# simensov/ml4ca

Hardware: AMD Instinct MI355X
Metric: env-steps/sec at 65536 parallel envs (higher is better)
Workload: dtype f32

## Files before the change

ml4ca_amd/csrc/dpenv_env_dev.h:

```cpp
#ifndef DPENV_ENV_DEV_H
#define DPENV_ENV_DEV_H
#include <hip/hip_runtime.h>
#include <hip/hip_bf16.h>
#include <stdint.h>

#include "dpenv_dev.h"

namespace dpenv {

constexpr float kPi = 3.14159265358979323846f;

__device__ __forceinline__ void philox4x32_10(uint32_t c0, uint32_t c1, uint32_t c2, uint32_t c3, uint32_t k0,
                                              uint32_t k1, uint32_t out[4])
{
#pragma unroll
    for (int r = 0; r < 10; ++r) {
        const uint64_t p0 = (uint64_t)c0 * 0xD2511F53ull, p1 = (uint64_t)c2 * 0xCD9E8D57ull;
        const uint32_t hi0 = (uint32_t)(p0 >> 32), lo0 = (uint32_t)p0, hi1 = (uint32_t)(p1 >> 32), lo1 = (uint32_t)p1;
        const uint32_t n0 = hi1 ^ c1 ^ k0, n2 = hi0 ^ c3 ^ k1;
        c0 = n0; c1 = lo1; c2 = n2; c3 = lo0;
        k0 += 0x9E3779B9u; k1 += 0xBB67AE85u;
    }
    out[0] = c0; out[1] = c1; out[2] = c2; out[3] = c3;
}
// ... 533 lines not shown
        if (live) {
            if (a.obs_bf16) {
                uint16_t* p = (uint16_t*)dst;
#pragma unroll
                for (int k = 0; k < OD; ++k) p[(int64_t)k * n + i] = f2bf(o[k]);
            } else {
                float* p = (float*)dst;
#pragma unroll
                for (int k = 0; k < OD; ++k) p[(int64_t)k * n + i] = o[k];
            }
        }
        return;
    }
    lds_order<BLOCK>();
#pragma unroll
    for (int k = 0; k < OD; ++k) lds[tid * OD + k] = o[k];
    lds_order<BLOCK>();
    const int64_t base = (int64_t)blockIdx.x * (BLOCK * OD);
    const int64_t rem = (int64_t)n * OD - base;
    store_rows<OD, BLOCK>(dst, base, rem, a.obs_bf16, lds, tid);
}

struct Env {
    float N, E, psi, u, v, r;
    float refN, refE, refPsi;
    float pt[3];
    float ang[3];
    int steps;
    float sn, cs;
};

struct StepOut {
    float o[9];
    float reward;
    float parts[4];
    uint32_t d;
};

struct Wrench {
    float thr[3];
    float tx, ty, tn;
};

template <int MODE, bool DEFER_ANG = false>
__device__ __forceinline__ void env_decode_cmd(float ang[3], const float* act, float thr[3])
{
    thr[0] = clipf(act[0] * 100.0f, 100.0f);
    thr[1] = clipf(act[1] * 100.0f, 100.0f);
    thr[2] = clipf(act[2] * 100.0f, 100.0f);
    if (MODE == MODE_FULL) {
        ang[0] = clipf(act[3] * kPi, kPi); ang[1] = clipf(act[4] * kPi, kPi); ang[2] = clipf(act[5] * kPi, kPi);
    } else if (MODE == MODE_LIMITED) {
        ang[1] = clipf(act[3] * (kPi * 0.5f), kPi * 0.5f); ang[2] = clipf(act[4] * (kPi * 0.5f), kPi * 0.5f);
    } else if (MODE == MODE_FINAL_WRAP) {
        const float w3 = act[3] - 2.0f * floorf((act[3] + 1.0f) * 0.5f);
        const float w4 = act[4] - 2.0f * floorf((act[4] + 1.0f) * 0.5f);
        ang[1] = clipf(w3 * kPi, kPi); ang[2] = clipf(w4 * kPi, kPi);
    } else if (MODE == MODE_FINAL_CONT) {
        if (!DEFER_ANG) { ang[1] = clipf(atan2_lean(act[3], act[4]), kPi); ang[2] = clipf(atan2_lean(act[5], act[6]), kPi); }
    }
}

template <int MODE, bool DEFER_ANG = false>
__device__ __forceinline__ void env_decode(const Vessel& ve, float ang[3], const float* act, Wrench& w, const ThrustLoss* tl = nullptr)
{
    env_decode_cmd<MODE, DEFER_ANG>(ang, act, w.thr);
    if (MODE == MODE_FINAL_CONT) {
        float sc[4];
        const float np2 = fmaf(act[3], act[3], act[4] * act[4]), ns2 = fmaf(act[5], act[5], act[6] * act[6]);
        const float ip = __builtin_amdgcn_rsqf(np2), is = __builtin_amdgcn_rsqf(ns2);
        sc[0] = (np2 > 0.0f) ? act[3] * ip : 0.0f; sc[1] = (np2 > 0.0f) ? act[4] * ip : 1.0f;
        sc[2] = (ns2 > 0.0f) ? act[5] * is : 0.0f; sc[3] = (ns2 > 0.0f) ? act[6] * is : 1.0f;
        thrust_map(ve, w.thr, ang, w.tx, w.ty, w.tn, sc, tl);
    } else {
        thrust_map(ve, w.thr, ang, w.tx, w.ty, w.tn, nullptr, tl);
    }
}

__device__ __forceinline__ void env_plant(const StepArgs& a, const Vessel& ve, float tx, float ty, float tn, bool cur, float vcN,
                                          float vcE, float& N, float& E, float& psi, float& u, float& v, float& r, float sn, float cs)
{
    if (cur) {
        u -= fmaf(cs, vcN, sn * vcE);
        v -= fmaf(cs, vcE, -(sn * vcN));
    }
    const float h = a.h;
    const float hA = h * ve.inv11, h22 = h * ve.i22, h23 = h * ve.i23, h33 = h * ve.i33;
    const float yur = ve.Yur + ve.m11;
    const float nuv = ve.Nuv - ve.m11;
    const int nsub = a.hold_plant ? 0 : a.n_substeps;
    float aN = 0.0f, aE = 0.0f;
#pragma unroll 10
    for (int k = 0; k < nsub; ++k) {
        const float q = fmaf(ve.m22, v, ve.m23 * r);
        float fx = fmaf(-fmaf(ve.Xuu, fabsf(u), ve.Xu), u, tx);
        fx = fmaf(q, r, fx);
        float fy = fmaf(-fmaf(ve.Yvv, fabsf(v), ve.Yv), v, ty);
        fy = fmaf(-fmaf(yur, u, ve.Yr), r, fy);
        float fn = fmaf(-q, u, tn);
        fn = fmaf(-fmaf(nuv, u, ve.Nv), v, fn);
        fn = fmaf(-fmaf(ve.Nrr, fabsf(r), ve.Nr), r, fn);
        u = fmaf(hA, fx, u);
        v = fmaf(h22, fy, fmaf(h23, fn, v));
        r = fmaf(h23, fy, fmaf(h33, fn, r));
        aN = fmaf(-sn, v, fmaf(cs, u, aN));
        aE = fmaf(cs, v, fmaf(sn, u, aE));
        const float d = h * r;
        const float e = -0.5f * d;
        psi += d;
        const float c2 = fmaf(fmaf(e, cs, -sn), d, cs);
        const float s2n = fmaf(fmaf(e, sn, cs), d, sn);
        cs = c2; sn = s2n;
    }
    N = fmaf(h, aN, N);
    E = fmaf(h, aE, E);
    if (cur) {
        const float hn = h * (float)nsub;
        N = fmaf(hn, vcN, N);
        E = fmaf(hn, vcE, E);
    }
}

__device__ __forceinline__ void env_plant_finish(bool cur, float vcN, float vcE, float se, float ce, float& u, float& v)
{
    if (cur) {
        u += fmaf(ce, vcN, se * vcE);
        v += fmaf(ce, vcE, -(se * vcN));
    }
}

template <int MODE, bool EXT>
__device__ __forceinline__ void env_reward(const StepArgs& a, const float* o, const float thr[3], const float pt_old[3],
                                           const float ang_new[3], const float ang_prev[3], StepOut& out)
{
    float p_der = 0.0f;
    const float p_vel = -sqrt_hw(fmaf(o[3] * o[3], 0.5f, fmaf(o[4] * o[4], 0.5f, o[5] * o[5])));
    const float rr2 = fmaf(o[0], o[0], o[1] * o[1]);
    const float yaw = o[2] * (180.0f / kPi);
    const float multivar = 2.0f * __builtin_amdgcn_exp2f((-0.5f * 1.4426950408889634f) * fmaf(yaw * yaw, 1.0f / 25.0f, rr2));
    const float special = sqrt_hw(fmaf(yaw * 0.25f, yaw * 0.25f, rr2));
    const float p_pos = multivar + fmaxf(-1.0f, fmaf(-0.1f, special, 1.0f)) + 0.5f;
    const float p_thr = -(fabsf(thr[0]) * 0.20f + fabsf(thr[1]) * 0.30f + fabsf(thr[2]) * 0.30f) * 0.01f;
    if (EXT) {
        const float inv_dt = a.inv_dt;
        float pen = 0.0f;
#pragma unroll
        for (int k = 0; k < 3; ++k) pen -= fabsf((thr[k] - pt_old[k]) * inv_dt * 0.01f) * 0.05f;
        const float inv_bnd = (MODE == MODE_LIMITED) ? (2.0f / kPi) : (1.0f / kPi);
        const float angpen = -(fabsf((ang_new[1] - ang_prev[1]) * inv_dt * inv_bnd) * 0.01f +
                               fabsf((ang_new[2] - ang_prev[2]) * inv_dt * inv_bnd) * 0.01f);
        p_der = pen + fmaxf(-1.0f, angpen);
    }
    out.parts[0] = p_vel; out.parts[1] = p_pos; out.parts[2] = p_thr; out.parts[3] = p_der;
    out.reward = p_vel + p_pos + p_thr + p_der;
}

template <int MODE>
__device__ __forceinline__ void env_done(const StepArgs& a, Env& s, const float* act, const float* o, const float thr[3], bool has_ref,
                                         float nrN, float nrE, float nrP, StepOut& out)
{
    uint32_t d = 0;
    if (a.terminate) {
        float b[6];
        ss_bounds<MODE>(b);
        bool t = false;
#pragma unroll
        for (int k = 0; k < 6; ++k) t = t || (fabsf(o[k]) > b[k]);
        d = t ? DONE_TERMINAL : 0u;
    }
    {
        float chk = s.N + s.E + s.psi + s.u + s.v + s.r;
#pragma unroll
        for (int k = 0; k < ModeTraits<MODE>::A; ++k) chk += act[k];
        if (!(fabsf(chk) <= 3.0e38f)) d |= DONE_TERMINAL | DONE_FAULT;
    }
    if (has_ref) { s.refN = nrN; s.refE = nrE; s.refPsi = nrP; }
    s.steps += 1;
    if (a.max_ep_len > 0 && s.steps >= a.max_ep_len) d |= DONE_TIMELIMIT;
    s.pt[0] = thr[0]; s.pt[1] = thr[1]; s.pt[2] = thr[2];
    out.d = d;
}

struct StepRest {
    float thr[3], pt_old[3], ang_prev[3], ang_new[3];
};

template <int MODE, bool EXT, bool DEFER>
__device__ __forceinline__ void env_step_chain(const StepArgs& a, const Vessel& ve, Env& s, const float* act, bool has_ref,
                                               float nrN, float nrE, float nrP, bool cur, float vcN, float vcE, StepOut& out, StepRest& rest,
                                               int il = -1)
{
#pragma unroll
    for (int k = 0; k < 3; ++k) { rest.ang_prev[k] = s.ang[k]; rest.pt_old[k] = s.pt[k]; }
    Wrench w;
    if (il == IL_SHARED || (il >= 0 && thrust_loss_on(a))) {
        ThrustLoss tl;
        if (il == IL_SHARED) {
#pragma unroll
            for (int k = 0; k < 3; ++k) { tl.klf[k] = a.kl[k]; tl.klr[k] = a.kl[3 + k]; }
        } else {
            const float4 q0 = a.env_tab[(int64_t)ENV_GROUPS * a.env_stride + il], q1 = a.env_tab[(int64_t)(ENV_GROUPS + 1) * a.env_stride + il];
            tl.klf[0] = q0.x; tl.klf[1] = q0.y; tl.klf[2] = q0.z; tl.klr[0] = q0.w; tl.klr[1] = q1.x; tl.klr[2] = q1.y;
        }
        tl.u = s.u; tl.v = s.v; tl.r = s.r;
        if (cur) {
            tl.u -= fmaf(s.cs, vcN, s.sn * vcE);
            tl.v -= fmaf(s.cs, vcE, -(s.sn * vcN));
        }
        env_decode<MODE, DEFER>(ve, s.ang, act, w, &tl);
    } else {
        env_decode<MODE, DEFER>(ve, s.ang, act, w);
    }
#pragma unroll
    for (int k = 0; k < 3; ++k) { rest.thr[k] = w.thr[k]; rest.ang_new[k] = s.ang[k]; }
    float N = s.N, E = s.E, psi = s.psi, u = s.u, v = s.v, r = s.r;
    env_plant(a, ve, w.tx, w.ty, w.tn, cur, vcN, vcE, N, E, psi, u, v, r, s.sn, s.cs);
    const bool deg = (a.wrap_mode == WRAP_REFERENCE);
    float* o = out.o;
    bool same;
    float se, ce;
    {
        make_obs(N, E, psi, 0.0f, 0.0f, 0.0f, s.refN, s.refE, s.refPsi, rest.pt_old, deg, o, se, ce, same);
        if (!same) sincos_lean(psi, se, ce);
    }
    env_plant_finish(cur, vcN, vcE, se, ce, u, v);
    o[3] = u; o[4] = v; o[5] = r;
    s.N = N; s.E = E; s.psi = psi; s.u = u; s.v = v; s.r = r;
    s.sn = se; s.cs = ce;
    env_done<MODE>(a, s, act, o, rest.thr, has_ref, nrN, nrE, nrP, out);
}

template <int MODE, bool EXT, bool DEFER>
__device__ __forceinline__ void env_step_finish(const StepArgs& a, Env& s, const float* act, StepRest& rest, bool untouched, StepOut& out)
{
    if (DEFER && MODE == MODE_FINAL_CONT) {
        rest.ang_new[1] = clipf(atan2_lean(act[3], act[4]), kPi);
        rest.ang_new[2] = clipf(atan2_lean(act[5], act[6]), kPi);
        if (untouched) { s.ang[1] = rest.ang_new[1]; s.ang[2] = rest.ang_new[2]; }
    }
    env_reward<MODE, EXT>(a, out.o, rest.thr, rest.pt_old, rest.ang_new, rest.ang_prev, out);
}

template <int MODE, bool EXT>
__device__ __forceinline__ void env_step(const StepArgs& a, const Vessel& ve, Env& s, const float* act, bool has_ref,
                                         float nrN, float nrE, float nrP, bool cur, float vcN, float vcE, StepOut& out, int il = -1)
{
    StepRest rest;
    env_step_chain<MODE, EXT, false>(a, ve, s, act, has_ref, nrN, nrE, nrP, cur, vcN, vcE, out, rest, il);
    env_step_finish<MODE, EXT, false>(a, s, act, rest, true, out);
}

struct ResetDraw {
    float eta[3], nu[3], pt[3];
};

template <int MODE>
__device__ __forceinline__ void reset_draw(const StepArgs& a, int64_t gid, uint32_t episode, ResetDraw& d)
{
    sample_reset<MODE>(a, gid, episode, d.eta, d.nu);
    d.pt[0] = d.pt[1] = d.pt[2] = 0.0f;
    if (a.reset_acts) sample_reset_thrust(a, gid, episode, d.pt);
}

template <int MODE>
__device__ __forceinline__ void reset_apply(const StepArgs& a, Env& s, const ResetDraw& d, float o_new[9])
{
    s.N = d.eta[0]; s.E = d.eta[1]; s.psi = d.eta[2]; s.u = d.nu[0]; s.v = d.nu[1]; s.r = d.nu[2];
    s.pt[0] = d.pt[0]; s.pt[1] = d.pt[1]; s.pt[2] = d.pt[2];
    default_angles<MODE>(s.ang[0], s.ang[1], s.ang[2]);
    s.steps = 0;
    bool same;
    make_obs(s.N, s.E, s.psi, s.u, s.v, s.r, s.refN, s.refE, s.refPsi, s.pt, a.wrap_mode == WRAP_REFERENCE, o_new, s.sn, s.cs,
             same);
    if (!same) sincos_lean(s.psi, s.sn, s.cs);
}

template <int MODE>
__device__ __forceinline__ void env_auto_reset(const StepArgs& a, Env& s, int64_t gid, uint32_t episode, float o_new[9])
{
    ResetDraw d;
    reset_draw<MODE>(a, gid, episode, d);
    reset_apply<MODE>(a, s, d, o_new);
}

__device__ __forceinline__ void load_env(const float4* S0, const float4* S1, const float4* S2, const float4* RF, int il, Env& s)
{
    const float4 s0 = S0[il], s1 = S1[il], s2 = S2[il], rf = RF[il];
    s.N = s0.x; s.E = s0.y; s.psi = s0.z; s.u = s0.w; s.v = s1.x; s.r = s1.y;
    s.ang[0] = rf.w; s.ang[1] = s1.z; s.ang[2] = s1.w;
    s.pt[0] = s2.x; s.pt[1] = s2.y; s.pt[2] = s2.z; s.steps = __float_as_int(s2.w);
    s.refN = rf.x; s.refE = rf.y; s.refPsi = rf.z;
}

__device__ __forceinline__ void load_env(const StepArgs& a, int il, Env& s) { load_env(a.S0, a.S1, a.S2, a.RF, il, s); }

__device__ __forceinline__ void store_env(const StepArgs& a, int i, const Env& s, bool rf_dirty)
{
    a.S0[i] = make_float4(s.N, s.E, s.psi, s.u);
    a.S1[i] = make_float4(s.v, s.r, s.ang[1], s.ang[2]);
    a.S2[i] = make_float4(s.pt[0], s.pt[1], s.pt[2], __int_as_float(s.steps));
    if (rf_dirty) a.RF[i] = make_float4(s.refN, s.refE, s.refPsi, s.ang[0]);
}

}

#endif
```

ml4ca_amd/csrc/dpenv_kernels.hip:

```cpp
#include "dpenv_env_dev.h"

namespace dpenv {

#ifdef DPENV_STEP_TRACE
__device__ uint32_t* g_step_trace = nullptr;
constexpr int STEP_TRACE_RING = 8;
#endif

constexpr int RESETW_FIELDS = 18;
constexpr int RESETW_FIELDS_RND = 20;

template <int MODE>
__device__ __forceinline__ void reset_wave(const StepArgs& a, float* lds, int lane, int blk)
{
    const int n = a.n;
    const int i = blk * 64 + lane;
    const int il = i < n ? i : n - 1;
    const uint32_t ep = (uint32_t)a.episode[il];
    const float4 rf = a.RF[il];
    Env s;
    s.refN = rf.x; s.refE = rf.y; s.refPsi = rf.z;
    if (a.new_ref) { s.refN = a.new_ref[il]; s.refE = a.new_ref[(int64_t)n + il]; s.refPsi = a.new_ref[2 * (int64_t)n + il]; }
    ResetDraw d;
    reset_draw<MODE>(a, a.env_id_base + i, ep, d);
    float o[9];
    reset_apply<MODE>(a, s, d, o);
    lds[0 * 64 + lane] = s.N; lds[1 * 64 + lane] = s.E; lds[2 * 64 + lane] = s.psi;
#pragma unroll
    for (int k = 0; k < 9; ++k) lds[(3 + k) * 64 + lane] = o[k];
    lds[12 * 64 + lane] = s.pt[0]; lds[13 * 64 + lane] = s.pt[1]; lds[14 * 64 + lane] = s.pt[2];
    lds[15 * 64 + lane] = s.sn; lds[16 * 64 + lane] = s.cs;
    lds[17 * 64 + lane] = __uint_as_float(ep);
}

template <int MODE>
__device__ __forceinline__ void reset_from_lds(const float* lds, int lane, Env& s, float o_new[9])
{
    s.N = lds[0 * 64 + lane]; s.E = lds[1 * 64 + lane]; s.psi = lds[2 * 64 + lane];
#pragma unroll
    for (int k = 0; k < 9; ++k) o_new[k] = lds[(3 + k) * 64 + lane];
    s.u = o_new[3]; s.v = o_new[4]; s.r = o_new[5];
    s.pt[0] = lds[12 * 64 + lane]; s.pt[1] = lds[13 * 64 + lane]; s.pt[2] = lds[14 * 64 + lane];
    default_angles<MODE>(s.ang[0], s.ang[1], s.ang[2]);
    s.steps = 0;
    s.sn = lds[15 * 64 + lane]; s.cs = lds[16 * 64 + lane];
}

template <int MODE, bool EXT, int VES, bool RESETW = false>
__global__ __launch_bounds__(RESETW ? 2 * BLOCK : BLOCK) void step_kernel(const StepArgs a)
{
    const float4 *pS0 = a.S0, *pS1 = a.S1, *pS2 = a.S2, *pRF = a.RF;
    const float* paction = a.action;
    const int pn = a.n, playout = a.action_layout;
    constexpr int A = ModeTraits<MODE>::A;
    constexpr int OD = EXT ? 9 : 6;
    constexpr bool PER_CLASS = VES == VES_CLASS_LDS;
    constexpr bool RND = VES == VES_ENV_RND;
    constexpr bool ENV_VGPR = VES == VES_ENV_VGPR || RND;
    constexpr int IL = VES == VES_ARGS_LOSS ? IL_SHARED : IL_NONE;
    constexpr bool CURR = RND || VES == VES_ARGS_LOSS;
    static_assert(!RESETW || BLOCK == 64, "the reset wave pairs with ONE env wave");
    static_assert(VES != VES_ENV_LDS || BLOCK == 64, "the LDS-DMA image is [group][lane] of one wave");
    __shared__ float lds_io[BLOCK * 9];
    __shared__ float lds_cls[PER_CLASS ? VD_COUNT * MAX_CLASSES : 1];
    __shared__ float4 lds_pe[VES == VES_ENV_LDS ? ENV_GROUPS * 64 : 1];
    __shared__ float lds_rst[RESETW ? (CURR ? RESETW_FIELDS_RND : RESETW_FIELDS) * 64 : 1];
    __shared__ uint32_t lds_fin[RESETW ? 64 : 1];

    if (RESETW && threadIdx.x >= BLOCK) {
        const int lane = threadIdx.x - BLOCK;
        reset_wave<MODE>(a, lds_rst, lane, blockIdx.x);
        float4 hull[DRAW_GROUPS];
        const int i = blockIdx.x * 64 + lane;
        const bool rnd = RND && a.rand_tab != nullptr;
        if (rnd)
            draw_env_groups(hull_key(a), a.env_id_base + i, __float_as_uint(lds_rst[17 * 64 + lane]), [&](int g, const float4& q) { hull[g] = q; });
        if (CURR && a.cur_nom) {
            const float2 cd = current_draw(a, i, i < a.n ? i : a.n - 1, __float_as_uint(lds_rst[17 * 64 + lane]));
            lds_rst[18 * 64 + lane] = cd.x; lds_rst[19 * 64 + lane] = cd.y;
        }
        __syncthreads();
        if (rnd && lds_fin[lane] != 0u) {
#pragma unroll
            for (int g = 0; g < DRAW_GROUPS; ++g) store_draw_group(a.env_tab, a.env_stride, i, g, hull[g]);
        }
        return;
    }
    const int tid = threadIdx.x;
    const int i = blockIdx.x * BLOCK + tid;
    const int n = pn;
    const bool live = i < n;
    const int il = live ? i : n - 1;
#ifdef DPENV_STEP_TRACE
    const uint64_t trace_t0 = wall_clock64();
#endif

    float act[A];
    if (playout == LAYOUT_AOS) {
        const int64_t base = (int64_t)blockIdx.x * (BLOCK * A);
        load_rows<A, BLOCK>(paction + base, (int64_t)n * A - base, tid, act);
    } else {
#pragma unroll
        for (int k = 0; k < A; ++k) act[k] = paction[(int64_t)k * n + il];
    }
    Env s;
    load_env(pS0, pS1, pS2, pRF, il, s);
    float nrN = 0.0f, nrE = 0.0f, nrP = 0.0f;
    if (a.new_ref) { nrN = a.new_ref[il]; nrE = a.new_ref[(int64_t)n + il]; nrP = a.new_ref[2 * (int64_t)n + il]; }
    Current cur = {0.0f, 0.0f, 0.0f, 0.0f, 0u};
    float vc0 = 0.0f, beta0 = 0.0f;
    if (a.cur_vc) {
        cur.vc = a.cur_vc[il]; cur.beta = a.cur_beta[il];
        if (a.current_drift) { vc0 = a.cur_vc0[il]; beta0 = a.cur_beta0[il]; cur.ctr = a.drift_ctr[il]; }
    }
    int cls = 0;
    if (PER_CLASS) cls = a.class_id[il];
    Vessel ve_env;
    if (ENV_VGPR) ve_env = vessel_from_env(a.env_tab, a.env_stride, il);
    if (VES == VES_ENV_LDS) {
#pragma unroll
        for (int g = 0; g < ENV_GROUPS; ++g)
            __builtin_amdgcn_global_load_lds((const __attribute__((address_space(1))) void*)(a.env_tab + ((int64_t)g * a.env_stride + il)),
                                             (__attribute__((address_space(3))) void*)(lds_pe + g * 64), 16, 0, 0);
    }
    __builtin_amdgcn_sched_barrier(0);
    sincos_lean(s.psi, s.sn, s.cs);
    if (a.cur_vc) current_components(cur);
    if (PER_CLASS) {
        for (int k = tid; k < VD_COUNT * a.n_classes; k += BLOCK) {
            const int c = k / VD_COUNT, p = k - c * VD_COUNT;
            lds_cls[p * a.n_classes + c] = a.class_tab[k];
        }
    }
    if (playout == LAYOUT_AOS) {
#pragma unroll
        for (int j = 0; j < A; ++j) lds_io[j * BLOCK + tid] = act[j];
    }
    if (playout == LAYOUT_AOS || PER_CLASS) lds_order<BLOCK>();
    if (playout == LAYOUT_AOS) {
#pragma unroll
        for (int k = 0; k < A; ++k) act[k] = lds_io[tid * A + k];
    }
    if (VES == VES_ENV_LDS) {
        asm volatile("s_waitcnt vmcnt(0)" ::: "memory");
        __builtin_amdgcn_wave_barrier();
    }
    const Vessel ve = ENV_VGPR ? ve_env : VES == VES_ENV_LDS ? vessel_from_env_lds(lds_pe, tid)
                    : PER_CLASS ? vessel_from_lds(lds_cls, a.n_classes, cls) : vessel_from_args(a.v0);

    StepOut out;
    StepRest rest;
    env_step_chain<MODE, EXT, false>(a, ve, s, act, a.new_ref != nullptr, nrN, nrE, nrP, a.cur_vc != nullptr, cur.vcN, cur.vcE, out, rest, RND ? il : IL);
    bool rf_dirty = (a.new_ref != nullptr) || (MODE == MODE_FULL);
#ifdef DPENV_STEP_TRACE
    const bool early = false;
#else
    const bool early = !RESETW && !a.auto_reset;
#endif
    if (early) {
        if (live) {
            if (EXT && a.S3) a.S3[i] = make_float4(out.o[6], out.o[7], out.o[8], 0.0f);
            store_env(a, i, s, rf_dirty);
            a.done[i] = (uint8_t)out.d;
        }
        __builtin_amdgcn_sched_barrier(0);
        store_obs<OD>(a, a.obs, out.o, i, live, lds_io);
        __builtin_amdgcn_sched_barrier(0);
    }
    env_step_finish<MODE, EXT, false>(a, s, act, rest, true, out);
    if (a.current_drift) {
        current_drift_step(a, cur, vc0, beta0, a.env_id_base + i);
        if (live) { a.cur_vc[i] = cur.vc; a.cur_beta[i] = cur.beta; a.drift_ctr[i] = cur.ctr; }
    }
    if (early) {
        if (live) {
            a.rew[i] = out.reward;
            if (a.parts) {
                a.parts[i] = out.parts[0]; a.parts[(int64_t)n + i] = out.parts[1];
                a.parts[2 * (int64_t)n + i] = out.parts[2]; a.parts[3 * (int64_t)n + i] = out.parts[3];
            }
        }
        return;
    }

    float o_next[9];
#pragma unroll
    for (int k = 0; k < 9; ++k) o_next[k] = out.o[k];

    if (RESETW) {
        lds_fin[tid] = (a.auto_reset && out.d != 0u && live) ? 1u : 0u;
        __syncthreads();
    }
    if (a.auto_reset && out.d != 0u && live) {
        if (a.final_obs) {
            for (int k = 0; k < OD; ++k) {
                const int64_t idx = (a.obs_layout == LAYOUT_SOA) ? (int64_t)k * n + i : (int64_t)i * OD + k;
                if (a.obs_bf16) ((uint16_t*)a.final_obs)[idx] = f2bf(out.o[k]);
                else ((float*)a.final_obs)[idx] = out.o[k];
            }
        }
        const uint32_t ep = RESETW ? __float_as_uint(lds_rst[17 * 64 + tid]) : (uint32_t)a.episode[i];
        a.episode[i] = (int)(ep + 1u);
        if (RESETW) {
            reset_from_lds<MODE>(lds_rst, tid, s, o_next);
            if (CURR && a.cur_nom) {
                const float v = lds_rst[18 * 64 + tid], b = lds_rst[19 * 64 + tid];
                a.cur_vc[i] = v; a.cur_beta[i] = b; a.cur_vc0[i] = v; a.cur_beta0[i] = b;
            }
        } else {
            env_auto_reset<MODE>(a, s, a.env_id_base + i, ep, o_next);
            if (RND && a.rand_tab) redraw_vessel_table(a, i, ep);
            if (CURR && a.cur_nom) {
                const float2 cd = current_draw(a, i, i, ep);
                a.cur_vc[i] = cd.x; a.cur_beta[i] = cd.y; a.cur_vc0[i] = cd.x; a.cur_beta0[i] = cd.y;
            }
        }
        rf_dirty = true;
    }

    if (live) {
        if (EXT && a.S3) a.S3[i] = make_float4(o_next[6], o_next[7], o_next[8], 0.0f);
        store_env(a, i, s, rf_dirty);
        a.rew[i] = out.reward;
        a.done[i] = (uint8_t)out.d;
        if (a.parts) {
            a.parts[i] = out.parts[0]; a.parts[(int64_t)n + i] = out.parts[1];
            a.parts[2 * (int64_t)n + i] = out.parts[2]; a.parts[3 * (int64_t)n + i] = out.parts[3];
        }
    }
    __builtin_amdgcn_sched_barrier(0);
    store_obs<OD>(a, a.obs, o_next, i, live, lds_io);
#ifdef DPENV_STEP_TRACE
    if (tid == 0 && g_step_trace) {
        const uint64_t t1 = wall_clock64();
        const uint32_t slot = (uint32_t)(s.steps - 1) % STEP_TRACE_RING;
        uint32_t* rec = g_step_trace + ((size_t)slot * gridDim.x + blockIdx.x) * 4;
        rec[0] = __builtin_amdgcn_s_getreg((31 << 11) | 20);
        rec[1] = __builtin_amdgcn_s_getreg((31 << 11) | 4);
        rec[2] = (uint32_t)trace_t0;
        rec[3] = (uint32_t)t1;
    }
#endif
}

template <int MODE, bool EXT, int VES>
__global__ __launch_bounds__(RBLOCK) void rollout_kernel(const StepArgs a, const RolloutArgs ra)
{
    constexpr int A = ModeTraits<MODE>::A;
    constexpr int OD = EXT ? 9 : 6;
    constexpr bool PER_CLASS = VES == VES_CLASS_LDS, RND = VES == VES_ENV_RND, PER_ENV = VES == VES_ENV_VGPR || RND;
    constexpr int IL = VES == VES_ARGS_LOSS ? IL_SHARED : IL_NONE;
    constexpr bool CURR = RND || VES == VES_ARGS_LOSS;
    __shared__ float lds_act[RBLOCK * 7];
    __shared__ float lds_obs[RBLOCK * 9];
    __shared__ float lds_cls[PER_CLASS ? VD_COUNT * MAX_CLASSES : 1];

    const int tid = threadIdx.x;
    const int i = blockIdx.x * RBLOCK + tid;
    const int n = a.n;
    const bool live = i < n;
    const int il = live ? i : n - 1;

    Env s;
    load_env(a, il, s);
    sincos_lean(s.psi, s.sn, s.cs);
    Current cur = {0.0f, 0.0f, 0.0f, 0.0f, 0u};
    float vc0 = 0.0f, beta0 = 0.0f;
    if (a.cur_vc) {
        cur.vc = a.cur_vc[il]; cur.beta = a.cur_beta[il];
        if (a.current_drift) { vc0 = a.cur_vc0[il]; beta0 = a.cur_beta0[il]; cur.ctr = a.drift_ctr[il]; }
        current_components(cur);
    }
    int cls = 0;
    if (PER_CLASS) {
        cls = a.class_id[il];
        for (int k = tid; k < VD_COUNT * a.n_classes; k += RBLOCK) {
            const int c = k / VD_COUNT, p = k - c * VD_COUNT;
            lds_cls[p * a.n_classes + c] = a.class_tab[k];
        }
        lds_order<RBLOCK>();
    }
    Vessel ve = PER_ENV ? vessel_from_env(a.env_tab, a.env_stride, il)
                        : (PER_CLASS ? vessel_from_lds(lds_cls, a.n_classes, cls) : vessel_from_args(a.v0));
    if (!PER_CLASS && !PER_ENV) pin_vessel_in_vgprs(ve);
    uint32_t episode = a.auto_reset ? (uint32_t)a.episode[il] : 0u;
    bool ep_dirty = false, rf_dirty = (MODE == MODE_FULL);

    const int64_t step_stride_act = (int64_t)n * A;
    const int64_t step_stride_obs = (int64_t)n * OD;
    const int64_t blk_act = (int64_t)blockIdx.x * (RBLOCK * A);
    const int64_t blk_obs = (int64_t)blockIdx.x * (RBLOCK * OD);

    float pre[A];
    auto fetch = [&](int t) {
        const float* src = ra.actions + (int64_t)t * step_stride_act;
        if (a.action_layout == LAYOUT_AOS) {
            load_rows<A, RBLOCK>(src + blk_act, step_stride_act - blk_act, tid, pre);
        } else {
#pragma unroll
            for (int k = 0; k < A; ++k) pre[k] = src[(int64_t)k * n + il];
        }
    };
    fetch(0);
    int next_switch = 0;
    bool cur_dirty = false;
    float lag[3] = {0.0f, 0.0f, 0.0f};
    for (int t = 0; t < ra.T; ++t) {
        float act[A];
        if (a.action_layout == LAYOUT_AOS) {
            lds_order<RBLOCK>();
#pragma unroll
            for (int j = 0; j < A; ++j) lds_act[j * RBLOCK + tid] = pre[j];
            lds_order<RBLOCK>();
#pragma unroll
            for (int k = 0; k < A; ++k) act[k] = lds_act[tid * A + k];
        } else {
#pragma unroll
            for (int k = 0; k < A; ++k) act[k] = pre[k];
        }
        if (t + 1 < ra.T) fetch(t + 1);

        bool has_ref = false;
        float nrN = 0.0f, nrE = 0.0f, nrP = 0.0f;
        if (next_switch < ra.n_switch && ra.switch_step[next_switch] == t) {
            const float* rp = ra.refs + (int64_t)next_switch * 3 * n;
            nrN = rp[il]; nrE = rp[(int64_t)n + il]; nrP = rp[2 * (int64_t)n + il];
            has_ref = true; rf_dirty = true;
            ++next_switch;
        }
        StepOut out;
        env_step<MODE, EXT>(a, ve, s, act, has_ref, nrN, nrE, nrP, a.cur_vc != nullptr, cur.vcN, cur.vcE, out, RND ? il : IL);
        if (a.current_drift) current_drift_step(a, cur, vc0, beta0, a.env_id_base + i);
        float o_next[9];
#pragma unroll
        for (int k = 0; k < 9; ++k) o_next[k] = out.o[k];
        if (a.auto_reset && out.d != 0u && live) {
            env_auto_reset<MODE>(a, s, a.env_id_base + i, episode, o_next);
            if (RND && a.rand_tab) redraw_vessel(a, i, episode, ve);
            if (CURR && a.cur_nom) { current_redraw_inline(a, i, episode, cur, vc0, beta0); cur_dirty = true; }
            ++episode; ep_dirty = true; rf_dirty = true;
        }
        lag[0] = o_next[6]; lag[1] = o_next[7]; lag[2] = o_next[8];
        if (live) {
            (ra.rew + (int64_t)t * n)[(unsigned)i] = out.reward;
            (ra.done + (int64_t)t * n)[(unsigned)i] = (uint8_t)out.d;
        }
        if (a.obs_layout == LAYOUT_SOA) {
            if (live) {
#pragma unroll
                for (int k = 0; k < OD; ++k) {
                    const int64_t idx = (int64_t)t * step_stride_obs + (int64_t)k * n + i;
                    if (a.obs_bf16) ((uint16_t*)ra.obs)[idx] = f2bf(o_next[k]);
                    else ((float*)ra.obs)[idx] = o_next[k];
                }
            }
        } else {
            lds_order<RBLOCK>();
#pragma unroll
            for (int k = 0; k < OD; ++k) lds_obs[tid * OD + k] = o_next[k];
            lds_order<RBLOCK>();
            store_rows<OD, RBLOCK>(ra.obs, (int64_t)t * step_stride_obs + blk_obs, step_stride_obs - blk_obs, a.obs_bf16,
                                   lds_obs, tid);
        }
    }
    if (live) {
        store_env(a, i, s, rf_dirty);
        if (EXT) a.S3[i] = make_float4(lag[0], lag[1], lag[2], 0.0f);
        if (ep_dirty) a.episode[i] = (int)episode;
        if (a.current_drift) { a.cur_vc[i] = cur.vc; a.cur_beta[i] = cur.beta; a.drift_ctr[i] = cur.ctr; }
        if (CURR && cur_dirty) store_current(a, i, cur, vc0, beta0, true);
    }
// ... 307 lines not shown
        float o[9];
        float sr_, cr_;
        bool same_;
        make_obs(s0.x, s0.y, s0.z, s0.w, s1.x, s1.y, rf.x, rf.y, rf.z, pt, a.wrap_mode == WRAP_REFERENCE, o, sr_, cr_, same_);
        store_obs<OD>(a, a.obs, o, i, live, lds_io);
    }
}

__global__ __launch_bounds__(BLOCK) void get_state_kernel(const StepArgs a, float* st, int32_t* ctr)
{
    const int i = blockIdx.x * BLOCK + threadIdx.x;
    const int64_t n = a.n;
    if (i >= a.n) return;
    const float4 s0 = a.S0[i], s1 = a.S1[i], s2 = a.S2[i], rf = a.RF[i];
    if (st) {
        st[0 * n + i] = s0.x; st[1 * n + i] = s0.y; st[2 * n + i] = s0.z;
        st[3 * n + i] = s0.w; st[4 * n + i] = s1.x; st[5 * n + i] = s1.y;
        st[6 * n + i] = rf.x; st[7 * n + i] = rf.y; st[8 * n + i] = rf.z;
        st[9 * n + i] = s2.x; st[10 * n + i] = s2.y; st[11 * n + i] = s2.z;
        st[12 * n + i] = rf.w; st[13 * n + i] = s1.z; st[14 * n + i] = s1.w;
    }
    if (ctr) { ctr[i] = __float_as_int(s2.w); ctr[n + i] = a.episode[i]; }
}

__global__ __launch_bounds__(BLOCK) void set_state_kernel(const StepArgs a, const float* st, const int32_t* ctr)
{
    const int i = blockIdx.x * BLOCK + threadIdx.x;
    const int64_t n = a.n;
    if (i >= a.n) return;
    float4 s2 = a.S2[i];
    if (st) {
        a.S0[i] = make_float4(st[0 * n + i], st[1 * n + i], st[2 * n + i], st[3 * n + i]);
        a.S1[i] = make_float4(st[4 * n + i], st[5 * n + i], st[13 * n + i], st[14 * n + i]);
        a.RF[i] = make_float4(st[6 * n + i], st[7 * n + i], st[8 * n + i], st[12 * n + i]);
        s2.x = st[9 * n + i]; s2.y = st[10 * n + i]; s2.z = st[11 * n + i];
        a.S3[i] = make_float4(s2.x * 0.01f, s2.y * 0.01f, s2.z * 0.01f, 0.0f);
    }
    if (ctr) { s2.w = __int_as_float(ctr[i]); a.episode[i] = ctr[n + i]; }
    a.S2[i] = s2;
}

__global__ __launch_bounds__(BLOCK) void pack_env_vessels_kernel(const float* raw, int64_t p_stride, int64_t i_stride, float4* tab, uint32_t* loss_flag,
                                                                 int stride, int n)
{
    const int i = blockIdx.x * BLOCK + threadIdx.x;
    if (i >= n) return;
    float r[RAND_NPARAM], d[ENV_BLOCK_FLOATS];
#pragma unroll
    for (int p = 0; p < RAND_NPARAM; ++p) r[p] = raw[p * p_stride + i * i_stride];
    derive_env_block(r, d);
    store_env_block(tab, stride, i, d);
    const bool bad = !(d[0] == d[0]);
    const float nanv = __builtin_nanf("");
    tab[(int64_t)ENV_GROUPS * stride + i] = bad ? make_float4(nanv, nanv, nanv, nanv) : make_float4(r[26], r[27], r[28], r[29]);
    tab[(int64_t)(ENV_GROUPS + 1) * stride + i] = bad ? make_float4(nanv, nanv, 0.0f, 0.0f) : make_float4(r[30], r[31], 0.0f, 0.0f);
    bool any = false;
#pragma unroll
    for (int p = 26; p < RAND_NPARAM; ++p) any = any || (r[p] != 0.0f);
    if (loss_flag && __ballot(any) != 0ull && (threadIdx.x & 63) == __builtin_ctzll(__ballot(true))) atomicOr(loss_flag, 1u);
}

__global__ __launch_bounds__(BLOCK) void unpack_env_vessels_kernel(const float4* tab, int stride, float* out, int n)
{
    const int i = blockIdx.x * BLOCK + threadIdx.x;
    if (i >= n) return;
    float d[ENV_BLOCK_FLOATS];
#pragma unroll
    for (int g = 0; g < ENV_GROUPS; ++g) {
        const float4 q = tab[(int64_t)g * stride + i];
        d[4 * g] = q.x; d[4 * g + 1] = q.y; d[4 * g + 2] = q.z; d[4 * g + 3] = q.w;
    }
    float r[32];
    r[0] = d[VD_M11]; r[1] = d[VD_M22]; r[2] = d[VD_M23]; r[3] = d[VD_M33];
    r[4] = d[VD_XU]; r[5] = d[VD_XUU]; r[6] = d[VD_YV]; r[7] = d[VD_YVV]; r[8] = d[VD_YR];
    r[9] = d[VD_NV]; r[10] = d[VD_NR]; r[11] = d[VD_NRR];
#pragma unroll
    for (int k = 0; k < 3; ++k) { r[12 + k] = d[VD_KF + k]; r[15 + k] = d[VD_KR + k]; r[18 + k] = d[VD_LX + k]; r[21 + k] = d[VD_LY + k]; }
    r[24] = d[VD_NUV]; r[25] = d[VD_YUR];
    {
        const float4 q0 = tab[(int64_t)ENV_GROUPS * stride + i], q1 = tab[(int64_t)(ENV_GROUPS + 1) * stride + i];
        r[26] = q0.x; r[27] = q0.y; r[28] = q0.z; r[29] = q0.w; r[30] = q1.x; r[31] = q1.y;
    }
#pragma unroll
    for (int p = 0; p < 32; ++p) out[(int64_t)p * n + i] = r[p];
}

__global__ __launch_bounds__(BLOCK) void thrust_map_kernel(const VesselDev vd, const float* n_pct, const float* alpha,
                                                           float* tau, int n)
{
    const int i = blockIdx.x * BLOCK + threadIdx.x;
    if (i >= n) return;
    const Vessel ve = vessel_from_args(vd);
    const float nn[3] = {n_pct[i], n_pct[(int64_t)n + i], n_pct[2 * (int64_t)n + i]};
    const float al[3] = {alpha[i], alpha[(int64_t)n + i], alpha[2 * (int64_t)n + i]};
    float tx, ty, tn;
    thrust_map(ve, nn, al, tx, ty, tn);
    tau[i] = tx; tau[(int64_t)n + i] = ty; tau[2 * (int64_t)n + i] = tn;
}


template <int V> struct GaeVec;
template <> struct GaeVec<2> { typedef float2 F; typedef uint16_t E; };
template <> struct GaeVec<1> { typedef float F; typedef uint8_t E; };

template <int V> struct GaeRow {
    typename GaeVec<V>::F r, v, b;
    typename GaeVec<V>::E e;
};

__device__ __forceinline__ float gae_get(const float2& x, int k) { return k == 0 ? x.x : x.y; }
__device__ __forceinline__ float gae_get(const float& x, int) { return x; }
__device__ __forceinline__ void gae_set(float2& x, int k, float v) { if (k == 0) x.x = v; else x.y = v; }
__device__ __forceinline__ void gae_set(float& x, int, float v) { x = v; }
__device__ __forceinline__ uint32_t gae_end(uint16_t e, int k) { return ((uint32_t)e >> (8 * k)) & 0xffu; }
__device__ __forceinline__ uint32_t gae_end(uint8_t e, int) { return e; }

__device__ __forceinline__ double wave_sum_fixed(double x)
{
#pragma unroll
    for (int off = 32; off > 0; off >>= 1) x += __shfl_down(x, off, 64);
    return x;
}

template <int V, int GAE_U>
__global__ __launch_bounds__(64) void gae_kernel(const float* __restrict__ rew, const float* __restrict__ val,
                                                 const uint8_t* __restrict__ end, const float* __restrict__ boot,
                                                 const float* __restrict__ last_val, int T, int n, float gamma, float lam,
                                                 float* __restrict__ adv, float* __restrict__ ret, double* __restrict__ partials)
{
    typedef typename GaeVec<V>::F F;
    typedef typename GaeVec<V>::E E;
    const int c0 = (blockIdx.x * 64 + threadIdx.x) * V;
    const bool live = c0 < n;
    const int cl = live ? c0 : 0;
    const float gl = gamma * lam;
    float acc[V], g[V], vnext[V];
#pragma unroll
    for (int k = 0; k < V; ++k) { acc[k] = 0.0f; g[k] = 0.0f; vnext[k] = 0.0f; }
    double s1 = 0.0, s2 = 0.0;
    F lv;
#pragma unroll
    for (int k = 0; k < V; ++k) gae_set(lv, k, 0.0f);
    if (last_val) lv = *(const F*)(last_val + cl);

    GaeRow<V> A[GAE_U], B[GAE_U];
    auto load = [&](GaeRow<V> (&buf)[GAE_U], int j) {
#pragma unroll
        for (int u = 0; u < GAE_U; ++u) {
            int t = T - 1 - j * GAE_U - u;
            t = t < 0 ? 0 : t;
            const int64_t k = (int64_t)t * n + cl;
            buf[u].r = *(const F*)(rew + k);
            buf[u].v = *(const F*)(val + k);
            if (boot) buf[u].b = *(const F*)(boot + k);
            if (end) buf[u].e = *(const E*)(end + k); else buf[u].e = 0;
        }
    };
    auto consume = [&](const GaeRow<V> (&buf)[GAE_U], int j) {
#pragma unroll
        for (int u = 0; u < GAE_U; ++u) {
            const int t = T - 1 - j * GAE_U - u;
            if (t < 0) break;
            F a_out, r_out;
#pragma unroll
            for (int k = 0; k < V; ++k) {
                const bool is_end = (t == T - 1) || (gae_end(buf[u].e, k) != 0u);
                if (is_end) {
                    const float l = boot ? gae_get(buf[u].b, k) : ((t == T - 1) ? gae_get(lv, k) : 0.0f);
                    acc[k] = 0.0f; g[k] = l; vnext[k] = l;
                }
                const float rk = gae_get(buf[u].r, k), vk = gae_get(buf[u].v, k);
                const float delta = rk + gamma * vnext[k] - vk;
                acc[k] = delta + gl * acc[k];
                g[k] = rk + gamma * g[k];
                vnext[k] = vk;
                gae_set(a_out, k, acc[k]);
                gae_set(r_out, k, g[k]);
                s1 += (double)acc[k];
                s2 += (double)acc[k] * (double)acc[k];
            }
            if (live) {
                const int64_t k = (int64_t)t * n + c0;
                *(F*)(adv + k) = a_out;
                *(F*)(ret + k) = r_out;
            }
        }
    };
    const int nb = (T + GAE_U - 1) / GAE_U;
    load(A, 0);
    for (int j = 0; j < nb; j += 2) {
        load(B, j + 1);
        consume(A, j);
        load(A, j + 2);
        consume(B, j + 1);
    }
    if (partials) {
        if (!live) { s1 = 0.0; s2 = 0.0; }
        s1 = wave_sum_fixed(s1);
        s2 = wave_sum_fixed(s2);
        if (threadIdx.x == 0) { partials[2 * blockIdx.x] = s1; partials[2 * blockIdx.x + 1] = s2; }
    }
}

__global__ __launch_bounds__(256) void gae_finalize_kernel(const double* __restrict__ partials, int nparts, double* __restrict__ out)
{
    __shared__ double red[2][256];
    double a = 0.0, b = 0.0;
    for (int k = threadIdx.x; k < nparts; k += 256) { a += partials[2 * k]; b += partials[2 * k + 1]; }
    red[0][threadIdx.x] = a; red[1][threadIdx.x] = b;
    __syncthreads();
    for (int w = 128; w > 0; w >>= 1) {
        if ((int)threadIdx.x < w) { red[0][threadIdx.x] += red[0][threadIdx.x + w]; red[1][threadIdx.x] += red[1][threadIdx.x + w]; }
        __syncthreads();
    }
    if (threadIdx.x == 0) { out[0] = red[0][0]; out[1] = red[1][0]; }
}

constexpr int SUMB = 256;
__global__ __launch_bounds__(SUMB) void sum_partial_kernel(const float* __restrict__ x, int64_t count, const float* mean, int squared,
                                                           double* __restrict__ partials)
{
    __shared__ double red[SUMB / 64];
    const float m = mean ? mean[0] : 0.0f;
    double s = 0.0;
    const int64_t nvec = ((reinterpret_cast<uintptr_t>(x) & 15u) == 0) ? count / 4 : 0;
    for (int64_t k = (int64_t)blockIdx.x * SUMB + threadIdx.x; k < nvec; k += (int64_t)gridDim.x * SUMB) {
        const float4 q = ((const float4*)x)[k];
        const float d0 = q.x - m, d1 = q.y - m, d2 = q.z - m, d3 = q.w - m;
        s += squared ? ((double)(d0 * d0) + (double)(d1 * d1) + (double)(d2 * d2) + (double)(d3 * d3))
                     : ((double)d0 + (double)d1 + (double)d2 + (double)d3);
    }
    for (int64_t k = nvec * 4 + (int64_t)blockIdx.x * SUMB + threadIdx.x; k < count; k += (int64_t)gridDim.x * SUMB) {
        const float d = x[k] - m;
        s += squared ? (double)(d * d) : (double)d;
    }
    s = wave_sum_fixed(s);
    if ((threadIdx.x & 63) == 0) red[threadIdx.x >> 6] = s;
    __syncthreads();
    if (threadIdx.x == 0) {
        double t = 0.0;
        for (int w = 0; w < SUMB / 64; ++w) t += red[w];
        partials[2 * blockIdx.x] = t; partials[2 * blockIdx.x + 1] = 0.0;
    }
}

__global__ __launch_bounds__(256) void sum_finalize_kernel(const double* __restrict__ partials, int nparts, float* __restrict__ out)
{
    __shared__ double red[256];
    double a = 0.0;
    for (int k = threadIdx.x; k < nparts; k += 256) a += partials[2 * k];
    red[threadIdx.x] = a;
    __syncthreads();
    for (int w = 128; w > 0; w >>= 1) {
        if ((int)threadIdx.x < w) red[threadIdx.x] += red[threadIdx.x + w];
        __syncthreads();
    }
    if (threadIdx.x == 0) out[0] = (float)red[0];
}

template <bool STATS>
__global__ __launch_bounds__(SUMB) void adv_apply_kernel(float* __restrict__ x, int64_t count, const float* mean, const float* std,
                                                         const double* stats, double total_count)
{
    float m, inv;
    if (STATS) {
        const double mu = stats[0] / total_count;
        double var = stats[1] / total_count - mu * mu;
        var = var > 0.0 ? var : 0.0;
        m = (float)mu;
        inv = 1.0f / ((float)sqrt(var) + 1e-8f);
    } else {
        m = mean[0];
        inv = 1.0f / (std[0] + 1e-8f);
    }
    const int64_t nvec = ((reinterpret_cast<uintptr_t>(x) & 15u) == 0) ? count / 4 : 0;
    for (int64_t k = (int64_t)blockIdx.x * SUMB + threadIdx.x; k < nvec; k += (int64_t)gridDim.x * SUMB) {
        float4 q = ((float4*)x)[k];
        q.x = (q.x - m) * inv; q.y = (q.y - m) * inv; q.z = (q.z - m) * inv; q.w = (q.w - m) * inv;
        ((float4*)x)[k] = q;
    }
    for (int64_t k = nvec * 4 + (int64_t)blockIdx.x * SUMB + threadIdx.x; k < count; k += (int64_t)gridDim.x * SUMB)
        x[k] = (x[k] - m) * inv;
}

constexpr int SUM_MAXGRID = 2048;
__device__ double g_sum_partials[2 * SUM_MAXGRID];

}

using namespace dpenv;

#ifdef DPENV_STEP_TRACE
extern "C" int dpenv_debug_set_step_trace(void* p)
{
    return (int)hipMemcpyToSymbol(HIP_SYMBOL(dpenv::g_step_trace), &p, sizeof p);
}
#endif

static bool vessel_source_ok(const StepArgs& a, int ves)
{
    return !(ves >= VES_ENV_VGPR && ves <= VES_ENV_RND && !a.env_tab) && (ves == VES_ARGS_LOSS) == (a.loss_on == LOSS_SHARED);
}

hipError_t dev::launch_step(const StepArgs* a, int mode, int ext, int ves, int reset_wave, hipStream_t s)
{
    if (!vessel_source_ok(*a, ves)) return hipErrorInvalidValue;
    const dim3 grid((a->n + BLOCK - 1) / BLOCK);
    const bool two = a->auto_reset && BLOCK == 64 && reset_wave;
    return with_mode_ext(mode, ext, [&](auto M, auto E) { return with_ves(ves, [&](auto V) {
        if (two) hipLaunchKernelGGL((step_kernel<M, E, step_ves(V), BLOCK == 64>), grid, dim3(2 * BLOCK), 0, s, *a);
        else hipLaunchKernelGGL((step_kernel<M, E, step_ves(V)>), grid, dim3(BLOCK), 0, s, *a);
        return hipGetLastError();
    }); });
}

hipError_t dev::launch_pack_env_vessels(const float* raw, int64_t p_stride, int64_t i_stride, float4* tab, uint32_t* loss_flag, int stride, int n,
                                        hipStream_t s)
{
    hipLaunchKernelGGL(pack_env_vessels_kernel, dim3((n + BLOCK - 1) / BLOCK), dim3(BLOCK), 0, s, raw, p_stride, i_stride, tab, loss_flag, stride, n);
    return hipGetLastError();
}

hipError_t dev::launch_unpack_env_vessels(const float4* tab, int stride, float* out, int n, hipStream_t s)
{
    hipLaunchKernelGGL(unpack_env_vessels_kernel, dim3((n + BLOCK - 1) / BLOCK), dim3(BLOCK), 0, s, tab, stride, out, n);
    return hipGetLastError();
}

hipError_t dev::launch_rollout(const StepArgs* a, const RolloutArgs* ra, int mode, int ext, int ves, int two_wave, hipStream_t s)
{
    if (!vessel_source_ok(*a, ves)) return hipErrorInvalidValue;
    const dim3 grid((a->n + RBLOCK - 1) / RBLOCK);
    return with_mode_ext(mode, ext, [&](auto M, auto E) { return with_ves(ves, [&](auto V) {
        if (two_wave) hipLaunchKernelGGL((rollout_ws_kernel<M, E, rollout_ves(V)>), grid, dim3(128), 0, s, *a, *ra);
        else hipLaunchKernelGGL((rollout_kernel<M, E, rollout_ves(V)>), grid, dim3(RBLOCK), 0, s, *a, *ra);
        return hipGetLastError();
    }); });
}

hipError_t dev::launch_reset(const StepArgs* a, int mode, int ext, const uint8_t* mask, const float* init, const float* ref, hipStream_t s)
{
    return with_mode_ext(mode, ext, [&](auto M, auto E) {
        hipLaunchKernelGGL((reset_kernel<M, E>), dim3((a->n + BLOCK - 1) / BLOCK), dim3(BLOCK), 0, s, *a, mask, init, ref);
        return hipGetLastError();
    });
}

hipError_t dev::launch_get_state(const StepArgs* a, float* st, int32_t* ctr, hipStream_t s)
{
    hipLaunchKernelGGL(get_state_kernel, dim3((a->n + BLOCK - 1) / BLOCK), dim3(BLOCK), 0, s, *a, st, ctr);
    return hipGetLastError();
}

hipError_t dev::launch_set_state(const StepArgs* a, const float* st, const int32_t* ctr, hipStream_t s)
{
    hipLaunchKernelGGL(set_state_kernel, dim3((a->n + BLOCK - 1) / BLOCK), dim3(BLOCK), 0, s, *a, st, ctr);
    return hipGetLastError();
}

hipError_t dev::launch_thrust_map(const VesselDev* vd, const float* n_pct, const float* alpha, float* tau, int n, hipStream_t s)
{
    hipLaunchKernelGGL(thrust_map_kernel, dim3((n + BLOCK - 1) / BLOCK), dim3(BLOCK), 0, s, *vd, n_pct, alpha, tau, n);
    return hipGetLastError();
}

int64_t dev::gae_workspace_bytes(int n)
{
    return (((int64_t)n + 63) / 64) * 2 * (int64_t)sizeof(double);
}

hipError_t dev::launch_gae(const float* rew, const float* val, const uint8_t* end, const float* boot, const float* last_val, int T, int n,
                           float gamma, float lam, float* adv, float* ret, double* workspace, double* stats, hipStream_t s)
{
    const uintptr_t al = reinterpret_cast<uintptr_t>(rew) | reinterpret_cast<uintptr_t>(val) | reinterpret_cast<uintptr_t>(adv) |
                         reinterpret_cast<uintptr_t>(ret) | reinterpret_cast<uintptr_t>(boot) | reinterpret_cast<uintptr_t>(last_val);
    const bool vec = (n % 2 == 0) && ((al & 7u) == 0) && ((reinterpret_cast<uintptr_t>(end) & 1u) == 0);
    const int lanes = vec ? n / 2 : n;
    const int grid = (lanes + 63) / 64;
    double* parts = stats ? workspace : nullptr;
    if (vec) hipLaunchKernelGGL((gae_kernel<2, 8>), dim3(grid), dim3(64), 0, s, rew, val, end, boot, last_val, T, n, gamma, lam, adv, ret, parts);
    else hipLaunchKernelGGL((gae_kernel<1, 8>), dim3(grid), dim3(64), 0, s, rew, val, end, boot, last_val, T, n, gamma, lam, adv, ret, parts);
    hipError_t e = hipGetLastError();
    if (e != hipSuccess || !stats) return e;
    hipLaunchKernelGGL(gae_finalize_kernel, dim3(1), dim3(256), 0, s, (const double*)parts, grid, stats);
    return hipGetLastError();
}

static int reduce_grid(int64_t count)
{
    int64_t g = (count / 4 + SUMB - 1) / SUMB;
    if (g > SUM_MAXGRID) g = SUM_MAXGRID;
    if (g < 1) g = 1;
    return (int)g;
}

hipError_t dev::launch_sum(const float* x, int64_t count, const float* mean, float* out, hipStream_t s)
{
    double* parts = nullptr;
    hipError_t e = hipGetSymbolAddress((void**)&parts, HIP_SYMBOL(g_sum_partials));
    if (e != hipSuccess) return e;
    const int grid = reduce_grid(count);
    hipLaunchKernelGGL(sum_partial_kernel, dim3(grid), dim3(SUMB), 0, s, x, count, mean, mean != nullptr ? 1 : 0, parts);
    hipLaunchKernelGGL(sum_finalize_kernel, dim3(1), dim3(256), 0, s, (const double*)parts, grid, out);
    return hipGetLastError();
}

hipError_t dev::launch_adv_apply(float* x, int64_t count, const float* mean, const float* std, const double* stats, double total_count,
                                 hipStream_t s)
{
    if (stats) hipLaunchKernelGGL(adv_apply_kernel<true>, dim3(reduce_grid(count)), dim3(SUMB), 0, s, x, count, mean, std, stats, total_count);
    else hipLaunchKernelGGL(adv_apply_kernel<false>, dim3(reduce_grid(count)), dim3(SUMB), 0, s, x, count, mean, std, stats, total_count);
    return hipGetLastError();
}
```

Measured before the change: 12.65 billion.

## Add lean step kernel path using buffer-resource loads and stores

```diff
diff --git a/ml4ca_amd/csrc/dpenv_env_dev.h b/ml4ca_amd/csrc/dpenv_env_dev.h
--- a/ml4ca_amd/csrc/dpenv_env_dev.h
+++ b/ml4ca_amd/csrc/dpenv_env_dev.h
@@ -859,6 +859,34 @@
     if (rf_dirty) a.RF[i] = make_float4(s.refN, s.refE, s.refPsi, s.ang[0]);
 }
 
+typedef uint32_t u32x4 __attribute__((ext_vector_type(4)));
+__device__ __forceinline__ __amdgpu_buffer_rsrc_t buf_rsrc(const void* p, uint32_t bytes)
+{
+    return __builtin_amdgcn_make_buffer_rsrc(const_cast<void*>(p), 0, (int)bytes, 0x00020000);
+}
+__device__ __forceinline__ float buf_load1(__amdgpu_buffer_rsrc_t r, uint32_t off)
+{
+    return __uint_as_float(__builtin_amdgcn_raw_buffer_load_b32(r, off, 0, 0));
+}
+__device__ __forceinline__ float4 buf_load4(__amdgpu_buffer_rsrc_t r, uint32_t off)
+{
+    const u32x4 q = __builtin_amdgcn_raw_buffer_load_b128(r, off, 0, 0);
+    return make_float4(__uint_as_float(q.x), __uint_as_float(q.y), __uint_as_float(q.z), __uint_as_float(q.w));
+}
+__device__ __forceinline__ void buf_store1(__amdgpu_buffer_rsrc_t r, uint32_t off, float x)
+{
+    __builtin_amdgcn_raw_buffer_store_b32(__float_as_uint(x), r, off, 0, 0);
+}
+__device__ __forceinline__ void buf_store4(__amdgpu_buffer_rsrc_t r, uint32_t off, float x, float y, float z, float w)
+{
+    const u32x4 q = {__float_as_uint(x), __float_as_uint(y), __float_as_uint(z), __float_as_uint(w)};
+    __builtin_amdgcn_raw_buffer_store_b128(q, r, off, 0, 0);
+}
+__device__ __forceinline__ void buf_store_u8(__amdgpu_buffer_rsrc_t r, uint32_t off, uint8_t x)
+{
+    __builtin_amdgcn_raw_buffer_store_b8(x, r, off, 0, 0);
+}
+
 }
 
 #endif
diff --git a/ml4ca_amd/csrc/dpenv_kernels.hip b/ml4ca_amd/csrc/dpenv_kernels.hip
--- a/ml4ca_amd/csrc/dpenv_kernels.hip
+++ b/ml4ca_amd/csrc/dpenv_kernels.hip
@@ -46,7 +46,68 @@
     s.sn = lds[15 * 64 + lane]; s.cs = lds[16 * 64 + lane];
 }
 
-template <int MODE, bool EXT, int VES, bool RESETW = false>
+template <int MODE, bool EXT>
+__device__ __forceinline__ void step_lean(const StepArgs& a, float* lds_io)
+{
+    constexpr int A = ModeTraits<MODE>::A;
+    constexpr int OD = EXT ? 9 : 6;
+    const int tid = threadIdx.x;
+    const uint32_t n = (uint32_t)a.n;
+    const uint32_t i = blockIdx.x * BLOCK + tid;
+    const uint32_t o16 = i * 16u, o4 = i * 4u;
+    const uint32_t oact = (blockIdx.x * (BLOCK * A) + tid) * 4u;
+    const uint32_t oobs = (blockIdx.x * (BLOCK * OD) + tid) * 4u;
+    const __amdgpu_buffer_rsrc_t rS0 = buf_rsrc(a.S0, n * 16u), rS1 = buf_rsrc(a.S1, n * 16u), rS2 = buf_rsrc(a.S2, n * 16u),
+                                 rRF = buf_rsrc(a.RF, n * 16u), rAct = buf_rsrc(a.action, n * (4u * A));
+
+    float act[A];
+#pragma unroll
+    for (int j = 0; j < A; ++j) act[j] = buf_load1(rAct, oact + j * (4u * BLOCK));
+    Env s;
+    {
+        const float4 s0 = buf_load4(rS0, o16), s1 = buf_load4(rS1, o16), s2 = buf_load4(rS2, o16), rf = buf_load4(rRF, o16);
+        s.N = s0.x; s.E = s0.y; s.psi = s0.z; s.u = s0.w; s.v = s1.x; s.r = s1.y;
+        s.ang[0] = rf.w; s.ang[1] = s1.z; s.ang[2] = s1.w;
+        s.pt[0] = s2.x; s.pt[1] = s2.y; s.pt[2] = s2.z; s.steps = __float_as_int(s2.w);
+        s.refN = rf.x; s.refE = rf.y; s.refPsi = rf.z;
+    }
+    const bool has_ref = a.new_ref != nullptr;
+    float nrN = 0.0f, nrE = 0.0f, nrP = 0.0f;
+    if (has_ref) {
+        const __amdgpu_buffer_rsrc_t rNR = buf_rsrc(a.new_ref, n * 12u);
+        nrN = buf_load1(rNR, o4); nrE = buf_load1(rNR, o4 + n * 4u); nrP = buf_load1(rNR, o4 + n * 8u);
+    }
+    __builtin_amdgcn_sched_barrier(0);
+    sincos_lean(s.psi, s.sn, s.cs);
+#pragma unroll
+    for (int j = 0; j < A; ++j) lds_io[j * BLOCK + tid] = act[j];
+    lds_order<BLOCK>();
+#pragma unroll
+    for (int k = 0; k < A; ++k) act[k] = lds_io[tid * A + k];
+    const Vessel ve = vessel_from_args(a.v0);
+
+    StepOut out;
+    StepRest rest;
+    env_step_chain<MODE, EXT, false>(a, ve, s, act, has_ref, nrN, nrE, nrP, false, 0.0f, 0.0f, out, rest, IL_NONE);
+    buf_store4(rS0, o16, s.N, s.E, s.psi, s.u);
+    buf_store4(rS1, o16, s.v, s.r, s.ang[1], s.ang[2]);
+    buf_store4(rS2, o16, s.pt[0], s.pt[1], s.pt[2], __int_as_float(s.steps));
+    if (has_ref || MODE == MODE_FULL) buf_store4(rRF, o16, s.refN, s.refE, s.refPsi, s.ang[0]);
+    buf_store_u8(buf_rsrc(a.done, n), i, (uint8_t)out.d);
+    __builtin_amdgcn_sched_barrier(0);
+    lds_order<BLOCK>();
+#pragma unroll
+    for (int k = 0; k < OD; ++k) lds_io[tid * OD + k] = out.o[k];
+    lds_order<BLOCK>();
+    const __amdgpu_buffer_rsrc_t rObs = buf_rsrc(a.obs, n * (4u * OD));
+#pragma unroll
+    for (int j = 0; j < OD; ++j) buf_store1(rObs, oobs + j * (4u * BLOCK), lds_io[j * BLOCK + tid]);
+    __builtin_amdgcn_sched_barrier(0);
+    env_step_finish<MODE, EXT, false>(a, s, act, rest, true, out);
+    buf_store1(buf_rsrc(a.rew, n * 4u), o4, out.reward);
+}
+
+template <int MODE, bool EXT, int VES, bool RESETW = false, bool LEAN = false>
 __global__ __launch_bounds__(RESETW ? 2 * BLOCK : BLOCK) void step_kernel(const StepArgs a)
 {
     const float4 *pS0 = a.S0, *pS1 = a.S1, *pS2 = a.S2, *pRF = a.RF;
@@ -66,7 +127,12 @@
     __shared__ float4 lds_pe[VES == VES_ENV_LDS ? ENV_GROUPS * 64 : 1];
     __shared__ float lds_rst[RESETW ? (CURR ? RESETW_FIELDS_RND : RESETW_FIELDS) * 64 : 1];
     __shared__ uint32_t lds_fin[RESETW ? 64 : 1];
-
+    static_assert(!LEAN || (VES == VES_ARGS && !RESETW), "the lean step takes its vessel from the arguments and has no reset wave");
+
+    if (LEAN) {
+        step_lean<MODE, EXT>(a, lds_io);
+        return;
+    }
     if (RESETW && threadIdx.x >= BLOCK) {
         const int lane = threadIdx.x - BLOCK;
         reset_wave<MODE>(a, lds_rst, lane, blockIdx.x);
@@ -980,16 +1046,33 @@
     return !(ves >= VES_ENV_VGPR && ves <= VES_ENV_RND && !a.env_tab) && (ves == VES_ARGS_LOSS) == (a.loss_on == LOSS_SHARED);
 }
 
+static bool step_lean_ok(const StepArgs& a, int ves)
+{
+#ifdef DPENV_STEP_TRACE
+    return false;
+#else
+    return ves == VES_ARGS && !a.auto_reset && !a.final_obs && !a.parts && !a.cur_vc && !a.current_drift && !a.S3 && !a.obs_bf16 &&
+           a.obs_layout == LAYOUT_AOS && a.action_layout == LAYOUT_AOS && (int64_t)a.n * 36 < ((int64_t)1 << 31);
+#endif
+}
+
 hipError_t dev::launch_step(const StepArgs* a, int mode, int ext, int ves, int reset_wave, hipStream_t s)
 {
     if (!vessel_source_ok(*a, ves)) return hipErrorInvalidValue;
     const dim3 grid((a->n + BLOCK - 1) / BLOCK);
     const bool two = a->auto_reset && BLOCK == 64 && reset_wave;
-    return with_mode_ext(mode, ext, [&](auto M, auto E) { return with_ves(ves, [&](auto V) {
-        if (two) hipLaunchKernelGGL((step_kernel<M, E, step_ves(V), BLOCK == 64>), grid, dim3(2 * BLOCK), 0, s, *a);
-        else hipLaunchKernelGGL((step_kernel<M, E, step_ves(V)>), grid, dim3(BLOCK), 0, s, *a);
-        return hipGetLastError();
-    }); });
+    const bool lean = step_lean_ok(*a, ves);
+    return with_mode_ext(mode, ext, [&](auto M, auto E) {
+        if (lean) {
+            hipLaunchKernelGGL((step_kernel<M, E, VES_ARGS, false, true>), grid, dim3(BLOCK), 0, s, *a);
+            return hipGetLastError();
+        }
+        return with_ves(ves, [&](auto V) {
+            if (two) hipLaunchKernelGGL((step_kernel<M, E, step_ves(V), BLOCK == 64>), grid, dim3(2 * BLOCK), 0, s, *a);
+            else hipLaunchKernelGGL((step_kernel<M, E, step_ves(V)>), grid, dim3(BLOCK), 0, s, *a);
+            return hipGetLastError();
+        });
+    });
 }
 
 hipError_t dev::launch_pack_env_vessels(const float* raw, int64_t p_stride, int64_t i_stride, float4* tab, uint32_t* loss_flag, int stride, int n,
```

After: 13.22 billion, median of 6. 1.04x the previous value.
